# maplant/mgf

Measured on AMD Instinct MI355X. Metric: contact_constraint_iters_per_sec, higher is better.
Workload: dtype f32

## Files before the change

mgf_amd/csrc/common.h:

```cpp
#pragma once
#include <hip/hip_runtime.h>
#include <stdint.h>
#include <stdio.h>
#include <string.h>

#include <string>
#include <vector>

#include "../../include/mgf_hip.h"

namespace mgf {

void set_error(const char* fmt, ...);

#define MGF_HIP_TRY(expr)                                                                  \
  do {                                                                                     \
    hipError_t _e = (expr);                                                                \
    if (_e != hipSuccess) {                                                                \
      mgf::set_error("%s failed: %s (%s:%d)", #expr, hipGetErrorString(_e), __FILE__, __LINE__); \
      return (_e == hipErrorOutOfMemory) ? MGF_ERR_OOM : MGF_ERR_HIP;                      \
    }                                                                                      \
  } while (0)

#define MGF_TRY(expr)                 \
// ... 54 lines not shown
  kWFrontier0 = 0, kWFrontier1 = 1, kWFrontier2 = 2,
  kWStackOverflow = 3,
  kWRowOverflow = 4,
  kWSolverAbort = 5,
  kWGridWide = 6,
  kWFlow5Fail = 7,
  kWTerrainWide = 8,
  kWFlow5MaxBlock = 9,
  kWRevRowOverflow = 10,
  kWNarrowMismatch = 11,
  kWStandbyBar = 12,
  kWSkipGuard = 14,
  kWF6MaxSlots = 16, kWF6MaxForeign = 17, kWF6Fail = 18, kWF6Edges = 19, kWF6EdgesBlock = 20,
  kWGhostCons = 21,
  kWBrickSlow = 22,
  kWLinksTicket = 23,
  kWBigPartsOverflow = 24,
  kWLast = kWBigPartsOverflow
};
constexpr int err_at(FlagWord k) { return (int)k - (int)kWStackOverflow; }

mgf_status prim_exclusive_scan_u32(mgf_ctx* ctx, const uint32_t* in, uint32_t* out, size_t n_plus_1);
mgf_status prim_sort_pairs_u32(mgf_ctx* ctx, const uint32_t* keys_in, uint32_t* keys_out, const uint32_t* vals_in, uint32_t* vals_out, size_t n,
                               unsigned end_bit);

}
```

mgf_amd/csrc/host_tick.inc:

```
enum TerrainPlan { kTerrainNone, kTerrainRows, kTerrainGrid };
static TerrainPlan terrain_plan(const mgf_world* w, bool two_pass) {
  if (two_pass || !w->terrain || w->terrain->m.tree.empty() || !w->n_owned) return kTerrainNone;
  return (w->terrain->grid.ready && !w->terrain_grid_off && !w->opt.terrain_tree && w->obstacles.empty()) ? kTerrainGrid : kTerrainRows;
}
static mgf_status world_integrate(mgf_world* w, float dt, bool complete, bool integrate, bool with_bounds, bool with_terrain_rows = false) {
  mgf_ctx* ctx = w->ctx;
  w->invalidate_tick_caches();
  if (w->n_owned == 0) return MGF_OK;
  SceneBounds* sb = with_bounds ? w->sb.p : nullptr;
  const uint32_t* guard = with_bounds ? w->word(kWSkipGuard) : nullptr;
  int* sb_part = (with_terrain_rows && integrate && with_bounds && !w->opt.no_fused_scene_bounds) ? w->sb_part.p : nullptr;
  w->bounds_cover = sb_part ? w->n_owned : 0u;
  MGF_TRY(w->bpk.ensure(4 * (size_t)std::max(w->n, w->n_owned), ctx->stream));
  w->pack_cover = integrate ? w->n_owned : 0u;
  CellSort cs;
  memset(&cs, 0, sizeof(cs));
  if (sb_part && w->plan.zero_launched && w->plan.n == w->n_owned && w->sbg_valid && w->opt.cells_in_integrate) {
    cs.grid = w->sb_grid.p; cs.shift = kMortonBits - 2 * (int)w->plan.levels; cs.min_frac = (float)w->opt.grid_min_frac_pct * 0.01f;
    cs.cell_of = w->cell_of.p; cs.rank = w->cell_rank.p; cs.cell_cnt = w->cell_cnt.p;
    w->cells_cover = w->n_owned; w->cells_levels = w->plan.levels;
  }
  WideSpec wd;
  memset(&wd, 0, sizeof(wd));
  w->wide_tick_on = false;
// ... 201 lines not shown
  if (w->cap_p == 0) { w->cap_p = std::max(4 * n, 1024u); w->cap_t = std::max(2 * n, 1024u); w->cap_c = std::max(4 * n, 1024u); }
  const uint32_t cap_p = w->cap_p, cap_c = w->cap_c;
  if (cap_p >= (1u << 27)) return fail(MGF_ERR_CAPACITY, "too many broadphase partners (k_count_contacts keeps a list position in 27 bits)");
  uint32_t levels = 4;
  const uint64_t cell_fill = (w->has_capsule && !w->has_compound && !w->opt.cell_fill_set) ? std::min<uint64_t>((uint64_t)w->opt.cell_fill, 8u) : (uint64_t)w->opt.cell_fill;
  while ((double)(cell_fill << (2 * levels)) * (double)w->grid_occupancy < 8.0 * (double)n && levels < (uint32_t)kMortonBits / 2) ++levels;
  const uint32_t cells = 1u << (2 * levels), nblocks = cells / kBlock;
  MGF_TRY(w->cell_of.ensure(n, s)); MGF_TRY(w->cell_rank.ensure(n, s)); MGF_TRY(w->sidx.ensure(n, s)); MGF_TRY(w->brank.ensure(n, s));
  w->list_generic = false;
  w->flow5_ok = true; w->flow5_prepped = false; w->flow6_prepped = false; w->f6_fail_known = false; w->canon_ready = false;
  w->scan_tiles = (uint32_t)(((size_t)std::max(cells, n) + 1 + kScanTile - 1) / kScanTile) + 1;
  MGF_TRY(w->scan_ws.ensure(3 * (2 * (size_t)w->scan_tiles + 2), s));
  MGF_TRY(w->cs_sums.ensure(3 * kCsSumStride, s)); MGF_TRY(w->tcn.ensure(n + 1, s)); MGF_TRY(w->front_cnt.ensure(2 * kTnRegions * kTnCntStride, s));
  MGF_TRY(w->lnodes.ensure(qlevel_offset(levels), s)); MGF_TRY(w->leaves.ensure(n, s));
  MGF_TRY(w->cell_lo.ensure((size_t)cells + 1, s)); MGF_TRY(w->cell_cnt.ensure((size_t)cells + 1, s));
  MGF_TRY(w->sub_lo.ensure(nblocks, s)); MGF_TRY(w->sub_hi.ensure(nblocks, s));
  MGF_TRY(w->sub2_lo.ensure(nblocks / 4 + 1, s)); MGF_TRY(w->sub2_hi.ensure(nblocks / 4 + 1, s));
  const bool rows_done = !early && w->terrain_rows_done;
  MGF_TRY(w->t_cnt.ensure(n + 1, s, rows_done, w->n_owned)); MGF_TRY(w->p_cnt.ensure(n + 1, s));
  MGF_TRY(w->t_off.ensure(n + 1, s)); MGF_TRY(w->p_off.ensure(n + 1, s));
  MGF_TRY(w->cons_nat.ensure(cap_c, s));
  MGF_TRY(links_ensure(w, cap_c));
  MGF_TRY(w->degb.ensure(n + 1, s)); MGF_TRY(w->rev.ensure((size_t)n * w->rev_cap, s));
  const bool bounds_done = !early && w->bounds_cover == n && n > 0;
  w->plan.levels = levels; w->plan.cells = cells; w->plan.n = n; w->plan.cap_c = cap_c; w->plan.solver_follows = solver_follows;
  {
    ZeroList z;
    memset(&z, 0, sizeof(z));
    z.p[0] = w->cell_cnt.p; z.words[0] = cells + 1;
    z.p[1] = w->t_cnt.p; z.words[1] = n + 1;
    if (rows_done) { z.p[1] = w->t_cnt.p + w->n_owned; z.words[1] = n - w->n_owned + 1; }
    z.p[2] = w->degb.p; z.words[2] = n + 1;
    z.p[3] = w->word(kWRevRowOverflow); z.words[3] = 1;
    z.p[4] = w->word(kWRowOverflow); z.words[4] = rows_done ? 0 : 1;
    z.p[5] = w->word(kWGridWide); z.words[5] = 1;
    z.p[6] = w->word(kWTerrainWide); z.words[6] = 1;
    z.p[7] = w->pair_stat.p; z.words[7] = kPairStatWords;
    z.p[16] = w->word(kWBrickSlow); z.words[16] = 1;
    z.p[17] = w->scan_ws.p; z.words[17] = 3 * (2 * w->scan_tiles + 2);
    z.p[18] = w->cs_sums.p; z.words[18] = ((early || !rows_done) ? 3 : 2) * kCsSumStride;
    z.p[20] = w->front_cnt.p; z.words[20] = 2 * kTnRegions * kTnCntStride;
    z.p[21] = w->word(kWBigPartsOverflow); z.words[21] = 1;
    z.p[19] = w->tcn.p; z.words[19] = n + 1;
    w->flow5_zeroed = false; w->flow6_zeroed = false;
    if (solver_follows && w->opt.solver_mode == 6) {
      bool ok = false;
      MGF_TRY(flow6_plan(w, cap_c, w->f6_prep_iters ? w->f6_prep_iters : 10u, &ok));
      if (ok) { flow6_zero_entries(w, cap_c, z, 8); w->flow6_zeroed = true; }
    }
    if (solver_follows && w->opt.solver_mode == 5) {
      bool ok = false;
      MGF_TRY(flow5_plan(w, cap_c, &ok));
      if (ok) { flow5_zero_entries(w, cap_c, z, 8); w->flow5_zeroed = true; }
// ... 213 lines not shown
}
static mgf_status stage_pair_search(mgf_world* w, const CollidePlan& P) {
  const Lbvh T = tick_tree(w, P);
  if (P.two_pass) {
    k_candidates<false><<<8 * xcd_blocks_per(P.n), kBlock, 0, P.s>>>(P.B, P.n, w->n_owned, T, P.M, 1e-3f, w->t_cnt.p, w->p_cnt.p, nullptr, nullptr, nullptr, nullptr, nullptr, nullptr, nullptr);
    LAUNCH_CHECK();
    if (P.n_obs && w->n_owned) {
      k_obstacle_candidates<false><<<nblk(w->n_owned), kBlock, 0, P.s>>>(P.B, w->n_owned, w->d_obs.p, P.n_obs, w->t_cnt.p, nullptr, nullptr, nullptr, nullptr);
      LAUNCH_CHECK();
    }
    return MGF_OK;
  }
  if (P.brick && !w->pair_brick_attr) {
    MGF_HIP_TRY(hipFuncSetAttribute(reinterpret_cast<const void*>(k_pair_brick<true>), hipFuncAttributeMaxDynamicSharedMemorySize, (int)brick_lds_bytes(true, kBrickCap)));
    MGF_HIP_TRY(hipFuncSetAttribute(reinterpret_cast<const void*>(k_pair_brick<false>), hipFuncAttributeMaxDynamicSharedMemorySize, (int)brick_lds_bytes(false, kBrickCap)));
    w->pair_brick_attr = true;
  }
  const uint32_t per_block = kCoopBlock / kCoopLanes;
  const uint32_t grid = 8 * (((P.n + per_block - 1) / per_block + 7) / 8);
  const uint32_t bricks = 8 * ((((1u << (2 * P.levels)) >> 6) + 7) / 8);
  uint32_t* const overflow = w->word(kWRowOverflow);
  uint32_t* const too_wide = w->word(kWGridWide);
  if (P.demo) {}
  else if (P.front_rows && w->has_compound) { MGF_TRY(w->cnt.ensure(P.n + 1, P.s)); k_pair_grid_n<true><<<grid, kCoopBlock, 0, P.s>>>(P.B, P.n, w->n_owned, T, w->sb.p, 1e-3f, w->rows.p, w->p_cnt.p, overflow, too_wide, w->pair_stat.p, P.min_frac, w->cnt.p); }
  else if (P.front_rows) k_pair_grid_n<false><<<grid, kCoopBlock, 0, P.s>>>(P.B, P.n, w->n_owned, T, w->sb.p, 1e-3f, w->rows.p, w->p_cnt.p, overflow, too_wide, w->pair_stat.p, P.min_frac, nullptr);
  else if (P.brick && P.fused) k_pair_brick<true><<<bricks, kCoopBlock, brick_lds_bytes(true, kBrickCap), P.s>>>(P.n, w->n_owned, T, w->rows.p, w->p_cnt.p, overflow, too_wide, w->pair_stat.p, w->word(kWBrickSlow), kBrickCap);
  else if (P.brick) k_pair_brick<false><<<bricks, kCoopBlock, brick_lds_bytes(false, kBrickCap), P.s>>>(P.n, w->n_owned, T, w->rows.p, w->p_cnt.p, overflow, too_wide, w->pair_stat.p, w->word(kWBrickSlow), kBrickCap);
  else if (P.use_grid && P.fused) k_pair_grid<true><<<grid, kCoopBlock, 0, P.s>>>(P.B, P.n, w->n_owned, T, w->sb.p, 1e-3f, w->rows.p, w->p_cnt.p, overflow, too_wide, w->pair_stat.p, P.min_frac);
  else if (P.use_grid) k_pair_grid<false><<<grid, kCoopBlock, 0, P.s>>>(P.B, P.n, w->n_owned, T, w->sb.p, 1e-3f, w->rows.p, w->p_cnt.p, overflow, too_wide, nullptr, P.min_frac);
  else k_pair_rows<<<grid, kCoopBlock, 0, P.s>>>(P.B, P.n, w->n_owned, T, 1e-3f, w->rows.p, w->p_cnt.p, overflow);
  LAUNCH_CHECK();
  if (P.wide_now) {
    PairWide W;
    W.list = w->wide_list.p; W.count = &w->sb.p->pad; W.T = T; W.sb = w->sb.p; W.box = P.grid_box_of; W.pad_abs = 1e-3f; W.min_frac = P.min_frac; W.n = P.n; W.n_owned = w->n_owned;
    W.contacts = (P.fused || P.front_rows) ? 1u : 0u; W.rows_p = w->rows.p; W.p_cnt = w->p_cnt.p; W.overflow = overflow; W.too_wide = too_wide;
    W.pair_stat = (P.fused || P.front_rows) ? w->pair_stat.p : nullptr; W.guard = w->word(kWSkipGuard);
    k_pair_wide<<<kWideCap, kBlock, 0, P.s>>>(P.B, W);
    LAUNCH_CHECK();
  }
  return MGF_OK;
}
static mgf_status contacts_from_rows(mgf_world* w, const CollidePlan& P, float dt) {
// ... 235 lines not shown
  {
    const SceneBounds* sbh = reinterpret_cast<SceneBounds*>(pin + mgf_world::kRbSb);
    float e[3], emax = 0.0f;
    for (int k = 0; k < 3; ++k) { e[k] = ord_f(sbh->hi[k]) - ord_f(sbh->lo[k]); emax = std::max(emax, e[k]); w->h_scene_ext[k] = e[k]; w->h_scene_rmax[k] = ord_f(sbh->rmax[k]); }
    const float mf = (float)w->opt.grid_min_frac_pct * 0.01f;
    float occ = 1.0f;
    const uint32_t P = 2u * std::max(w->plan.levels, 4u), nbh[3] = {(P + 2u) / 3u, (P + 1u) / 3u, P / 3u};
    if (emax > 0.0f && mf > 0.0f) for (int k = 0; k < 3; ++k) if (e[k] < mf * emax) {
      const float wide = std::max(e[k], std::min(mf * emax, 1.36f * w->h_scene_rmax[k] * (float)(1u << nbh[k])));
      occ *= std::max(e[k], 1e-3f * emax) / wide;
    }
    w->grid_occupancy = (occ > 0.0f && occ <= 1.0f) ? std::max(occ, 0.3f) : 1.0f;
  }
  w->wide_last = w->wide_tick_on ? reinterpret_cast<SceneBounds*>(pin + mgf_world::kRbSb)->pad : 0u;
  w->pair_brick_slow = w->ts->brick ? w->ts->word(kWBrickSlow) : 0;
  if (w->ts->brick) {
    if (w->pair_brick_slow * 32 > (uint64_t)w->n + 1024) { w->pair_brick_off = w->pair_brick_backoff; w->pair_brick_backoff = std::min(2u * w->pair_brick_backoff, 1u << 20); }
    else w->pair_brick_backoff = 256;
  }
  w->f6_fail_known = w->flow6_prepped; w->f6_fail_host = w->ts->word(kWF6Fail);
  w->f6_edges_block = w->flow6_prepped ? w->ts->word(kWF6EdgesBlock) : 0u;
  w->rb_fresh = true;
  if (w->ts->word(kWStackOverflow)) return fail(MGF_ERR_CAPACITY, "BVH traversal stack overflow");
  if (w->ts->word(kWBigPartsOverflow)) return fail(MGF_ERR_CAPACITY, "two bodies of many components meet in more than 64 part pairs or a manifold of more than 16 contacts (k_narrow_pairs_big)");
  if (w->ts->word(kWNarrowMismatch)) return fail(MGF_ERR_HIP, "internal error: the broadphase's sphere test and the constraint setup disagree about a contact");
  auto grown = [](uint32_t need) { return (uint32_t)std::min<uint64_t>((uint64_t)need + need / 2 + 1024, 0x7FFFFFF0ull); };
  if (h.fail & kFailSkipped) { *retry = true; return MGF_OK; }
  if (h.fail & kFailRevRow) { w->rev_cap *= 2; *retry = true; }
  if (h.fail & kFailFlow6) {
    const uint32_t slots = w->ts->word(kWF6MaxSlots), foreign = w->ts->word(kWF6MaxForeign);
// ... 102 lines not shown
```

mgf_amd/csrc/host_world.inc:

```
struct WorldOptions {
  int64_t resort_every = -1;
  int64_t grid_min_frac_pct = 50;
  int64_t cell_fill = 16;
  bool cell_fill_set = false;
  int64_t cells_in_integrate = 1;
  int64_t no_fused_scene_bounds = 0;
  int64_t no_fused_terrain_rows = 0;
  int64_t two_pass = 0;
  int64_t terrain_tree = 0;
  int64_t broadphase_tree = 0;
  int64_t pair_brick = 1;
  int64_t no_fused_narrowphase = 0;
  int64_t fused_contacts = 1;
  int64_t front_rows = 1;
  int64_t front_rows_check = 0;
  int64_t side_stream = 1;
  int64_t wide_list = 1;
  int64_t constraint_order = 0;
  int64_t solver_mode = 6;
  int64_t flow_spin_limit = 0;
  int64_t flow_max_blocks = 0;
  int64_t flow_trace = 0;
  int64_t flow5_block = 0;
  int64_t flow5_test_cap = 0;
  int64_t flow6_fcap = 0;
  int64_t flow6_spec_wl = -1;
  int64_t flow6_spec = 0;
  int64_t flow6_poll_waves = 0;
  int64_t flow6_const_lds = 1;
  int64_t flow6_foreign_lds = 1;
  int64_t flow6_quad = 1;
  int64_t flow6_quad_max = -1;
  int64_t flow6_slot_margin = 0;
  int64_t flow6_rec_lds = 1;
  int64_t flow6_nimp_lds = 1;
  int64_t flow6_test_cap = 0;
  int64_t pipeline = 1;
  int64_t readback_kernel = 1;
// ... 51 lines not shown
  bool wide_engaged = false, wide_tick_on = false;
  float wide_ref[3] = {0, 0, 0}, wide_limit[3] = {0, 0, 0};
  float shape_rmax[3] = {0, 0, 0};
  uint32_t wide_hold = 0, wide_last = 0;
  uint64_t n_wide_ticks = 0, n_wide_overflows = 0;
  uint64_t n_path_ticks[7] = {0, 0, 0, 0, 0, 0, 0};
  DBuf<float4> wide_list;
  DBuf<float4> q_bc, q_br;
  DBuf<uint32_t> q_cnt, q_start, q_items, q_large, q_misc, q_off, q_vals;
  DBuf<ParticleIn> q_parts; DBuf<int32_t> q_ign, q_hits; DBuf<float> q_boxes;
  DBuf<MovingIn> q_casts;
  uint32_t q_last_large = 0, q_last_cells = 0;
  float q_last_build_ms = 0.0f, q_last_run_ms = 0.0f;
  bool front_rows_off = false;
  uint64_t pair_brick_slow = 0;
  uint32_t pair_brick_off = 0;
  uint32_t pair_brick_backoff = 256;
  bool pair_brick_attr = false;
  DBuf<float4> sub_lo, sub_hi, sub2_lo, sub2_hi;
  DBuf<uint32_t> cell_lo, cell_cnt;
  DBuf<uint32_t> t_cnt, p_cnt, t_off, p_off, t_cand, t_owner, p_cand, p_owner, rows, rows_t;
  DBuf<uint32_t> flow_arr, flow_arr5;
  DBuf<uint64_t> flow_trace;
  DBuf<uint32_t> brank, f5_shared, f5_gcnt, f5_lslot, f5_wg_cnt;
  DBuf<F5Row> f5_table;
  bool flow5_zeroed = false;
  bool f6_fail_known = false;
  uint32_t f6_fail_host = 0;
  bool f6_standby = false;
  uint32_t f6_edges_block = 0;
  bool links_ready = false;
  bool flow5_ok = false, flow5_prepped = false;
  uint32_t f5_nb = 0, f5_nblocks = 0;
  DBuf<uint4> f6_binfo;
  DBuf<uint32_t> f6_bref, f6_fcnt, f6_fbody, f6_nslots, f6_in_key, f6_in_cnt, f6_out_key, f6_out_val, f6_chan_prefix;
// ... 197 lines not shown
  ctx_release(ctx);
}
extern "C" int64_t mgf_world_len(const mgf_world* w) { return w ? (int64_t)w->n_owned : 0; }

struct OptionEntry { const char* key; int64_t WorldOptions::*field; int64_t lo, hi; const char* range; bool plan, prep; };
static const OptionEntry kOptionTable[] = {
    {"time_solver_kernels", &WorldOptions::time_solver_kernels, 1, 0, nullptr, false, false},
    {"two_pass_candidates", &WorldOptions::two_pass, 1, 0, nullptr, true, false},
    {"broadphase_tree", &WorldOptions::broadphase_tree, 1, 0, nullptr, true, false},
    {"terrain_tree", &WorldOptions::terrain_tree, 1, 0, nullptr, true, false},
    {"no_fused_scene_bounds", &WorldOptions::no_fused_scene_bounds, 1, 0, nullptr, true, false},
    {"no_fused_terrain_rows", &WorldOptions::no_fused_terrain_rows, 1, 0, nullptr, true, false},
    {"grid_min_frac_pct", &WorldOptions::grid_min_frac_pct, 0, 100, "grid_min_frac_pct: 0..100", true, false},
    {"no_fused_narrowphase", &WorldOptions::no_fused_narrowphase, 1, 0, nullptr, false, false},
    {"pair_brick", &WorldOptions::pair_brick, 1, 0, nullptr, false, false},
    {"fused_contacts", &WorldOptions::fused_contacts, 1, 0, nullptr, false, false},
    {"front_rows", &WorldOptions::front_rows, 1, 0, nullptr, false, false},
    {"front_rows_check", &WorldOptions::front_rows_check, 1, 0, nullptr, false, false},
    {"side_stream", &WorldOptions::side_stream, 1, 0, nullptr, false, false},
    {"cells_in_integrate", &WorldOptions::cells_in_integrate, 1, 0, nullptr, false, false},
    {"solver_mode", &WorldOptions::solver_mode, 1, 0, nullptr, false, true},
    {"flow_trace", &WorldOptions::flow_trace, 1, 0, nullptr, false, false},
    {"flow_spin_limit", &WorldOptions::flow_spin_limit, 0, 4 << 20, "flow_spin_limit: 0 .. 4194304", false, false},
    {"flow5_test_cap", &WorldOptions::flow5_test_cap, 1, 0, nullptr, false, false},
    {"flow6_fcap", &WorldOptions::flow6_fcap, 0, 1536, "flow6_fcap out of range", false, false},
    {"flow6_const_lds", &WorldOptions::flow6_const_lds, 1, 0, nullptr, false, false},
    {"flow6_foreign_lds", &WorldOptions::flow6_foreign_lds, 1, 0, nullptr, false, false},
    {"flow6_nimp_lds", &WorldOptions::flow6_nimp_lds, 1, 0, nullptr, false, false},
    {"flow6_rec_lds", &WorldOptions::flow6_rec_lds, 1, 0, nullptr, false, false},
    {"flow6_slot_margin", &WorldOptions::flow6_slot_margin, 0, 1024, "flow6_slot_margin: 0..1024", false, false},
// ... 61 lines not shown
      w->has_compound = true;
    }
    return MGF_OK;
  }
  if (!strcmp(key, "list_capacity")) {
    if (value < 1 || value > 0x7FFFFFF0ll) return fail(MGF_ERR_INVALID, "list_capacity out of range");
    w->cap_t = w->cap_p = w->cap_c = (uint32_t)value;
    return MGF_OK;
  }
  return fail(MGF_ERR_INVALID, "unknown option");
}

extern "C" mgf_status mgf_world_counter(const mgf_world* w, const char* name, int64_t* out) {
  if (!w || !name || !out) return fail(MGF_ERR_INVALID, "NULL argument");
  if (!strcmp(name, "pair_brick_slow_queries")) { *out = (int64_t)w->pair_brick_slow; return MGF_OK; }
  if (!strcmp(name, "pair_brick_off_ticks")) { *out = (int64_t)w->pair_brick_off; return MGF_OK; }
  if (!strncmp(name, "scene_rmax_milli_", 17) && name[17] >= 'x' && name[17] <= 'z' && !name[18]) { *out = (int64_t)std::ceil((double)w->h_scene_rmax[name[17] - 'x'] * 1000.0); return MGF_OK; }
  if (!strncmp(name, "scene_ext_milli_", 16) && name[16] >= 'x' && name[16] <= 'z' && !name[17]) { *out = (int64_t)std::ceil((double)w->h_scene_ext[name[16] - 'x'] * 1000.0); return MGF_OK; }
  if (!strcmp(name, "grid_levels")) { *out = (int64_t)w->plan.levels; return MGF_OK; }
  if (!strcmp(name, "max_fat_half_extent_x_milli")) { *out = (int64_t)std::ceil((double)w->last_rmax_x * 1000.0); return MGF_OK; }
  if (!strncmp(name, "cross_probe_", 12)) {
    *out = 0;
    mgf_world* mw = const_cast<mgf_world*>(w);
    const size_t n = w->n;
    if (!w->constraints_ready || w->C == 0 || n == 0) return MGF_OK;
    MGF_TRY(ctx_bind(mw->ctx));
    std::vector<float4> x(n);
    MGF_TRY(d2h(mw->ctx, x.data(), mw->x.p, n));
    float lo[3] = {3e38f, 3e38f, 3e38f}, hi[3] = {-3e38f, -3e38f, -3e38f};
    for (const float4& v : x) { const float c[3] = {v.x, v.y, v.z}; for (int k = 0; k < 3; ++k) { lo[k] = std::min(lo[k], c[k]); hi[k] = std::max(hi[k], c[k]); } }
// ... 594 lines not shown
```

mgf_amd/csrc/k_broadphase.h:

```cpp
#pragma once
#include "k_bodies.h"

namespace mgf {

__device__ __forceinline__ uint32_t expand10(uint32_t v) {
  v = (v * 0x00010001u) & 0xFF0000FFu;
  v = (v * 0x00000101u) & 0x0F00F00Fu;
  v = (v * 0x00000011u) & 0xC30C30C3u;
  v = (v * 0x00000005u) & 0x49249249u;
  return v;
}
__device__ __forceinline__ uint32_t morton_quant(float v, float lo, float hi) {
  float ext = hi - lo;
  float t = ext > 0.0f ? (v - lo) / ext : 0.0f;
  int qv = (int)(t * 1023.0f);
  return (uint32_t)(qv < 0 ? 0 : (qv > 1023 ? 1023 : qv));
}
__device__ __forceinline__ uint32_t face_cell(uint32_t cx, uint32_t cy, uint32_t cz, uint3 bits) {
  return (((cx << bits.y) | cy) << bits.z) | cz;
}
constexpr int kMortonBits = 30;
constexpr float kBodyGridMinFrac = 0.5f;
__device__ __forceinline__ void grid_box(const SceneBounds* sb, float min_frac, uint32_t P, float* lo, float* hi) {
  float ext = 0.0f;
// ... 1022 lines not shown
    if (!SPHERES && np > (uint32_t)kRowCap) atomicOr(overflow, 1u);
  }
  if (SPHERES) {
    __shared__ uint32_t s_sum;
    if (threadIdx.x == 0) s_sum = 0;
    __syncthreads();
    uint32_t v = (live && sub == 0) ? n_accepted : 0u;
#pragma unroll
    for (int o = 32; o >= 1; o >>= 1) v += __shfl_xor(v, o);
    if (lane == 0 && v) atomicAdd(&s_sum, v);
    __syncthreads();
    if (threadIdx.x == 0 && s_sum) atomicAdd(&pair_stat[blockIdx.x & (kPairStatWords - 1u)], s_sum);
  }
}

template <bool SPHERES>
__global__ __launch_bounds__(kCoopBlock) __attribute__((amdgpu_waves_per_eu(6, 8))) void k_pair_brick(uint32_t n, uint32_t n_owned, Lbvh T,
                                                           uint32_t* rows_p, uint32_t* p_cnt, uint32_t* overflow, uint32_t* too_wide,
                                                           uint32_t* pair_stat, uint32_t* slow_queries, uint32_t cap) {
  extern __shared__ float4 s_dyn[];
  __shared__ uint16_t s_start[516];
  __shared__ uint32_t s_wsum[kCoopBlock / 64];
  __shared__ uint16_t s_acc[SPHERES ? kBrickQueries : 1][SPHERES ? kRowCap : 1];
  __shared__ uint32_t s_cnt[kBrickQueries][3];
  __shared__ uint32_t s_qo[kBrickQueries];
  __shared__ uint32_t s_sum, s_slow, s_q[2];
  const uint32_t P = 2u * T.levels;
  const uint32_t nbricks = (1u << P) >> 6;
  const uint32_t brick = xcd_logical_block_coop();
  if (brick >= nbricks) return;
  const uint32_t nb[3] = {(P + 2u) / 3u, (P + 1u) / 3u, P / 3u};
  const int shift = kMortonBits - (int)P;
  BrickSrcLds L;
  const uint32_t capp = brick_phys_cap(cap);
// ... 17 lines not shown
    }
  }
  if (t == 0) { s_sum = 0; s_slow = 0; }
  uint32_t inc = cnt;
#pragma unroll
  for (int o = 1; o < 64; o <<= 1) { uint32_t u = __shfl_up(inc, o); if (lane >= o) inc += u; }
  if (lane == 63) s_wsum[t >> 6] = inc;
  if (t == ((2u << 6) | (2u << 3) | 2u)) s_q[0] = g0;
  if (t == ((5u << 6) | (5u << 3) | 5u)) s_q[1] = g0 + cnt;
  __syncthreads();
  const uint32_t q0 = s_q[0], q1 = s_q[1];
  if (q0 == q1) return;
  uint32_t base = 0, total = 0;
#pragma unroll
  for (int w = 0; w < kCoopBlock / 64; ++w) { const uint32_t u = s_wsum[w]; if (w < (int)(t >> 6)) base += u; total += u; }
  const uint32_t start = base + inc - cnt;
  const bool staged = total <= cap;
  s_start[t] = (uint16_t)min(start, 0xFFFFu);
  if (t == 0) { s_start[512] = (uint16_t)min(total, 0xFFFFu); s_start[513] = s_start[512]; }
  uint32_t kq = q0 + t / (uint32_t)kBrickLanes;
  float4 qc, qr, qa, qv;
  qc = qr = qa = qv = make_float4(0, 0, 0, 0);
  uint32_t qi = 0;
  uint2 qreg = make_uint2(0, 0);
  if (kq < q1) { qc = T.ltb[2 * kq]; qr = T.ltb[2 * kq + 1]; if (SPHERES) { qa = T.lcol[2 * kq]; qv = T.lcol[2 * kq + 1]; } qi = T.sidx[kq]; qreg = make_uint2(f2u(qc.w), f2u(qr.w)); }
  if ((t & (uint32_t)(kBrickLanes - 1)) == 0u) s_qo[t / (uint32_t)kBrickLanes] = kq < q1 ? f2u(T.leaves[kq].r.w) : 0u;
  if (staged) {
    float4* rc = s_dyn; float4* rr = s_dyn + capp; float4* cc = s_dyn + 2 * capp; float4* cd = s_dyn + 3 * capp;
    for (uint32_t r = 0; r < cnt; ++r) {
      LeafRec lr = T.leaves[g0 + r];
      const uint32_t pp = brick_phys(start + r);
      rc[pp] = lr.c; rr[pp] = lr.r;
      if (SPHERES) { cc[pp] = T.lcol[2 * (g0 + r)]; cd[pp] = T.lcol[2 * (g0 + r) + 1]; }
    }
  }
  __syncthreads();
  const uint32_t sub = t & (uint32_t)(kBrickLanes - 1), qg = t / (uint32_t)kBrickLanes;
  uint32_t acc_total = 0, slow = 0;
  for (;;) {
    const bool live = kq < q1;
    const uint32_t i = qi, oi = s_qo[qg];
    uint32_t np = 0;
    if (sub == 0) { s_cnt[qg][0] = 0; s_cnt[qg][1] = 0; s_cnt[qg][2] = 0; }
    __builtin_amdgcn_fence(__ATOMIC_ACQ_REL, "wavefront");
    if (live && oi != 0 && T.n >= 2) {
      Box q; q.c = xyz(qc); q.r = xyz(qr);
      Comp A; A.p = xyz(qa); A.r = qa.w; A.d = mk3(0, 0, 0); A.kind = KIND_SPHERE;
      const V3 vA = xyz(qv);
      const uint32_t ca[3] = {qreg.x & 1023u, (qreg.x >> 10) & 1023u, qreg.x >> 20}, d[3] = {qreg.y & 1023u, (qreg.y >> 10) & 1023u, qreg.y >> 20};
      uint32_t* row = rows_p + (size_t)i * kRowCap;
      if (d[0] * d[1] * d[2] > kGridMaxCells) {
        if (sub == 0) *too_wide = 1u;
      } else if (staged && (int)ca[0] >= L.hb[0] && (int)ca[1] >= L.hb[1] && (int)ca[2] >= L.hb[2] && (int)(ca[0] + d[0]) <= L.hb[0] + 8 &&
                 (int)(ca[1] + d[1]) <= L.hb[1] + 8 && (int)(ca[2] + d[2]) <= L.hb[2] + 8) {
        brick_query<SPHERES>(L, q, A, vA, oi, n_owned, ca, d, sub, (uint32_t)kBrickLanes, row, s_acc[SPHERES ? qg : 0], s_cnt[qg]);
      } else if (sub == 0) {
        BrickSrcGlobal S; S.T = T; S.nb[0] = nb[0]; S.nb[1] = nb[1]; S.nb[2] = nb[2]; S.shift = shift;
        brick_query<SPHERES>(S, q, A, vA, oi, n_owned, ca, d, 0u, 1u, row, row, s_cnt[qg]);
        ++slow;
      }
      __builtin_amdgcn_fence(__ATOMIC_ACQ_REL, "wavefront");
      const uint32_t accepted = *(volatile uint32_t*)&s_cnt[qg][0];
      np = SPHERES ? *(volatile uint32_t*)&s_cnt[qg][2] : accepted;
      if (sub == 0) {
        acc_total += accepted;
        if (accepted > (uint32_t)kRowCap) atomicOr(overflow, 1u);
      }
    }
    if (live && sub == 0) p_cnt[i] = np;
    kq += kBrickQueries;
    if (kq - qg >= q1) break;
    qi = 0;
    if (kq < q1) { qc = T.ltb[2 * kq]; qr = T.ltb[2 * kq + 1]; if (SPHERES) { qa = T.lcol[2 * kq]; qv = T.lcol[2 * kq + 1]; } qi = T.sidx[kq]; qreg = make_uint2(f2u(qc.w), f2u(qr.w)); }
    if (sub == 0) s_qo[qg] = kq < q1 ? f2u(T.leaves[kq].r.w) : 0u;
  }
  {
    uint32_t v = acc_total, u = slow;
#pragma unroll
    for (int o = 32; o >= 1; o >>= 1) { v += __shfl_xor(v, o); u += __shfl_xor(u, o); }
    if (lane == 0 && v) atomicAdd(&s_sum, v);
    if (lane == 0 && u) atomicAdd(&s_slow, u);
    __syncthreads();
    if (SPHERES && t == 0 && s_sum) atomicAdd(&pair_stat[blockIdx.x & (kPairStatWords - 1u)], s_sum);
    if (t == 0 && s_slow) atomicAdd(slow_queries, s_slow);
  }
}
constexpr size_t brick_lds_bytes(bool spheres, uint32_t cap) { return (size_t)brick_phys_cap(cap) * 16u * (spheres ? 4u : 2u); }

struct FaceGrid {
  Lbvh T;
  uint3 bits;
  const SceneBounds* sb;
  const uint32_t* rank_of_face;
  const uint32_t* leaf_of_face;
  const uint32_t* parent;
};
__global__ __launch_bounds__(kCoopBlock) void k_terrain_grid(Bodies B, uint32_t n_owned, const uint32_t* order, TerrainDev M, FaceGrid G,
                                                             float pad_abs, uint32_t cap_row, uint32_t* rows_t, uint32_t* t_cnt,
                                                             uint32_t* overflow, uint32_t* too_wide) {
  const int lane = threadIdx.x & 63;
  const int sub = lane & 7;
// ... 132 lines not shown
```

Before: 8.422 billion.

## Split overfull bricks into sub-brick LDS passes instead of per-lane global fallback

Bricks whose staged leaf count exceeds LDS capacity no longer fall back to slow single-lane global-memory queries. They are appended to an overflow list and handled by a second kernel. That kernel splits each brick into Morton sub-ranges small enough to stage in LDS and serves their queries cooperatively. The cost is an extra kernel launch every tick, more counter words, and added complexity in the sub-range partitioning.

```diff
diff --git a/mgf_amd/csrc/common.h b/mgf_amd/csrc/common.h
--- a/mgf_amd/csrc/common.h
+++ b/mgf_amd/csrc/common.h
@@ -92,8 +92,11 @@
   kWF6MaxSlots = 16, kWF6MaxForeign = 17, kWF6Fail = 18, kWF6Edges = 19, kWF6EdgesBlock = 20,
   kWGhostCons = 21,
   kWBrickSlow = 22,
-  kWLinksTicket = 23,
-  kWBigPartsOverflow = 24,
+  kWBrickSplit = 23,
+  kWBrickLane = 24,
+  kWBrickOver = 25,
+  kWLinksTicket = 26,
+  kWBigPartsOverflow = 27,
   kWLast = kWBigPartsOverflow
 };
 constexpr int err_at(FlagWord k) { return (int)k - (int)kWStackOverflow; }
diff --git a/mgf_amd/csrc/host_tick.inc b/mgf_amd/csrc/host_tick.inc
--- a/mgf_amd/csrc/host_tick.inc
+++ b/mgf_amd/csrc/host_tick.inc
@@ -239,6 +239,7 @@
   MGF_TRY(w->cs_sums.ensure(3 * kCsSumStride, s)); MGF_TRY(w->tcn.ensure(n + 1, s)); MGF_TRY(w->front_cnt.ensure(2 * kTnRegions * kTnCntStride, s));
   MGF_TRY(w->lnodes.ensure(qlevel_offset(levels), s)); MGF_TRY(w->leaves.ensure(n, s));
   MGF_TRY(w->cell_lo.ensure((size_t)cells + 1, s)); MGF_TRY(w->cell_cnt.ensure((size_t)cells + 1, s));
+  MGF_TRY(w->brick_over.ensure((size_t)cells / 64 + 8, s));
   MGF_TRY(w->sub_lo.ensure(nblocks, s)); MGF_TRY(w->sub_hi.ensure(nblocks, s));
   MGF_TRY(w->sub2_lo.ensure(nblocks / 4 + 1, s)); MGF_TRY(w->sub2_hi.ensure(nblocks / 4 + 1, s));
   const bool rows_done = !early && w->terrain_rows_done;
@@ -261,7 +262,7 @@
     z.p[5] = w->word(kWGridWide); z.words[5] = 1;
     z.p[6] = w->word(kWTerrainWide); z.words[6] = 1;
     z.p[7] = w->pair_stat.p; z.words[7] = kPairStatWords;
-    z.p[16] = w->word(kWBrickSlow); z.words[16] = 1;
+    z.p[16] = w->word(kWBrickSlow); z.words[16] = 4;
     z.p[17] = w->scan_ws.p; z.words[17] = 3 * (2 * w->scan_tiles + 2);
     z.p[18] = w->cs_sums.p; z.words[18] = ((early || !rows_done) ? 3 : 2) * kCsSumStride;
     z.p[20] = w->front_cnt.p; z.words[20] = 2 * kTnRegions * kTnCntStride;
@@ -505,18 +506,27 @@
   if (P.brick && !w->pair_brick_attr) {
     MGF_HIP_TRY(hipFuncSetAttribute(reinterpret_cast<const void*>(k_pair_brick<true>), hipFuncAttributeMaxDynamicSharedMemorySize, (int)brick_lds_bytes(true, kBrickCap)));
     MGF_HIP_TRY(hipFuncSetAttribute(reinterpret_cast<const void*>(k_pair_brick<false>), hipFuncAttributeMaxDynamicSharedMemorySize, (int)brick_lds_bytes(false, kBrickCap)));
+    MGF_HIP_TRY(hipFuncSetAttribute(reinterpret_cast<const void*>(k_pair_brick_split<true>), hipFuncAttributeMaxDynamicSharedMemorySize, (int)brick_lds_bytes(true, kBrickCap)));
+    MGF_HIP_TRY(hipFuncSetAttribute(reinterpret_cast<const void*>(k_pair_brick_split<false>), hipFuncAttributeMaxDynamicSharedMemorySize, (int)brick_lds_bytes(false, kBrickCap)));
     w->pair_brick_attr = true;
   }
   const uint32_t per_block = kCoopBlock / kCoopLanes;
   const uint32_t grid = 8 * (((P.n + per_block - 1) / per_block + 7) / 8);
   const uint32_t bricks = 8 * ((((1u << (2 * P.levels)) >> 6) + 7) / 8);
+  static_assert(kWBrickSplit == kWBrickSlow + 1 && kWBrickLane == kWBrickSlow + 2 && kWBrickOver == kWBrickSlow + 3, "k_pair_brick and k_pair_brick_split count into four consecutive words");
+  const uint32_t brick_cap = w->opt.pair_brick_test_cap > 0 ? (uint32_t)std::min<int64_t>(w->opt.pair_brick_test_cap, (int64_t)kBrickCap) : kBrickCap;
   uint32_t* const overflow = w->word(kWRowOverflow);
   uint32_t* const too_wide = w->word(kWGridWide);
   if (P.demo) {}
   else if (P.front_rows && w->has_compound) { MGF_TRY(w->cnt.ensure(P.n + 1, P.s)); k_pair_grid_n<true><<<grid, kCoopBlock, 0, P.s>>>(P.B, P.n, w->n_owned, T, w->sb.p, 1e-3f, w->rows.p, w->p_cnt.p, overflow, too_wide, w->pair_stat.p, P.min_frac, w->cnt.p); }
   else if (P.front_rows) k_pair_grid_n<false><<<grid, kCoopBlock, 0, P.s>>>(P.B, P.n, w->n_owned, T, w->sb.p, 1e-3f, w->rows.p, w->p_cnt.p, overflow, too_wide, w->pair_stat.p, P.min_frac, nullptr);
-  else if (P.brick && P.fused) k_pair_brick<true><<<bricks, kCoopBlock, brick_lds_bytes(true, kBrickCap), P.s>>>(P.n, w->n_owned, T, w->rows.p, w->p_cnt.p, overflow, too_wide, w->pair_stat.p, w->word(kWBrickSlow), kBrickCap);
-  else if (P.brick) k_pair_brick<false><<<bricks, kCoopBlock, brick_lds_bytes(false, kBrickCap), P.s>>>(P.n, w->n_owned, T, w->rows.p, w->p_cnt.p, overflow, too_wide, w->pair_stat.p, w->word(kWBrickSlow), kBrickCap);
+  else if (P.brick && P.fused) {
+    k_pair_brick<true><<<bricks, kCoopBlock, brick_lds_bytes(true, kBrickCap), P.s>>>(P.n, w->n_owned, T, w->rows.p, w->p_cnt.p, overflow, too_wide, w->pair_stat.p, w->word(kWBrickSlow), brick_cap, w->brick_over.p);
+    k_pair_brick_split<true><<<std::min(bricks, kBrickSplitBlocks), kCoopBlock, brick_lds_bytes(true, kBrickCap), P.s>>>(w->n_owned, T, w->rows.p, w->p_cnt.p, overflow, too_wide, w->pair_stat.p, w->word(kWBrickSlow), brick_cap, w->brick_over.p);
+  } else if (P.brick) {
+    k_pair_brick<false><<<bricks, kCoopBlock, brick_lds_bytes(false, kBrickCap), P.s>>>(P.n, w->n_owned, T, w->rows.p, w->p_cnt.p, overflow, too_wide, w->pair_stat.p, w->word(kWBrickSlow), brick_cap, w->brick_over.p);
+    k_pair_brick_split<false><<<std::min(bricks, kBrickSplitBlocks), kCoopBlock, brick_lds_bytes(false, kBrickCap), P.s>>>(w->n_owned, T, w->rows.p, w->p_cnt.p, overflow, too_wide, w->pair_stat.p, w->word(kWBrickSlow), brick_cap, w->brick_over.p);
+  }
   else if (P.use_grid && P.fused) k_pair_grid<true><<<grid, kCoopBlock, 0, P.s>>>(P.B, P.n, w->n_owned, T, w->sb.p, 1e-3f, w->rows.p, w->p_cnt.p, overflow, too_wide, w->pair_stat.p, P.min_frac);
   else if (P.use_grid) k_pair_grid<false><<<grid, kCoopBlock, 0, P.s>>>(P.B, P.n, w->n_owned, T, w->sb.p, 1e-3f, w->rows.p, w->p_cnt.p, overflow, too_wide, nullptr, P.min_frac);
   else k_pair_rows<<<grid, kCoopBlock, 0, P.s>>>(P.B, P.n, w->n_owned, T, 1e-3f, w->rows.p, w->p_cnt.p, overflow);
@@ -782,6 +792,8 @@
   }
   w->wide_last = w->wide_tick_on ? reinterpret_cast<SceneBounds*>(pin + mgf_world::kRbSb)->pad : 0u;
   w->pair_brick_slow = w->ts->brick ? w->ts->word(kWBrickSlow) : 0;
+  w->pair_brick_split = w->ts->brick ? w->ts->word(kWBrickSplit) : 0;
+  w->pair_brick_lane = w->ts->brick ? w->ts->word(kWBrickLane) : 0;
   if (w->ts->brick) {
     if (w->pair_brick_slow * 32 > (uint64_t)w->n + 1024) { w->pair_brick_off = w->pair_brick_backoff; w->pair_brick_backoff = std::min(2u * w->pair_brick_backoff, 1u << 20); }
     else w->pair_brick_backoff = 256;
diff --git a/mgf_amd/csrc/host_world.inc b/mgf_amd/csrc/host_world.inc
--- a/mgf_amd/csrc/host_world.inc
+++ b/mgf_amd/csrc/host_world.inc
@@ -22,6 +22,7 @@
   int64_t flow_max_blocks = 0;
   int64_t flow_trace = 0;
   int64_t flow5_block = 0;
+  int64_t pair_brick_test_cap = 0;
   int64_t flow5_test_cap = 0;
   int64_t flow6_fcap = 0;
   int64_t flow6_spec_wl = -1;
@@ -103,11 +104,14 @@
   float q_last_build_ms = 0.0f, q_last_run_ms = 0.0f;
   bool front_rows_off = false;
   uint64_t pair_brick_slow = 0;
+  uint64_t pair_brick_split = 0;
+  uint64_t pair_brick_lane = 0;
   uint32_t pair_brick_off = 0;
   uint32_t pair_brick_backoff = 256;
   bool pair_brick_attr = false;
   DBuf<float4> sub_lo, sub_hi, sub2_lo, sub2_hi;
   DBuf<uint32_t> cell_lo, cell_cnt;
+  DBuf<uint32_t> brick_over;
   DBuf<uint32_t> t_cnt, p_cnt, t_off, p_off, t_cand, t_owner, p_cand, p_owner, rows, rows_t;
   DBuf<uint32_t> flow_arr, flow_arr5;
   DBuf<uint64_t> flow_trace;
@@ -335,6 +339,7 @@
     {"grid_min_frac_pct", &WorldOptions::grid_min_frac_pct, 0, 100, "grid_min_frac_pct: 0..100", true, false},
     {"no_fused_narrowphase", &WorldOptions::no_fused_narrowphase, 1, 0, nullptr, false, false},
     {"pair_brick", &WorldOptions::pair_brick, 1, 0, nullptr, false, false},
+    {"pair_brick_test_cap", &WorldOptions::pair_brick_test_cap, 1, 0, nullptr, false, false},
     {"fused_contacts", &WorldOptions::fused_contacts, 1, 0, nullptr, false, false},
     {"front_rows", &WorldOptions::front_rows, 1, 0, nullptr, false, false},
     {"front_rows_check", &WorldOptions::front_rows_check, 1, 0, nullptr, false, false},
@@ -426,6 +431,8 @@
 extern "C" mgf_status mgf_world_counter(const mgf_world* w, const char* name, int64_t* out) {
   if (!w || !name || !out) return fail(MGF_ERR_INVALID, "NULL argument");
   if (!strcmp(name, "pair_brick_slow_queries")) { *out = (int64_t)w->pair_brick_slow; return MGF_OK; }
+  if (!strcmp(name, "pair_brick_split_queries")) { *out = (int64_t)w->pair_brick_split; return MGF_OK; }
+  if (!strcmp(name, "pair_brick_lane_queries")) { *out = (int64_t)w->pair_brick_lane; return MGF_OK; }
   if (!strcmp(name, "pair_brick_off_ticks")) { *out = (int64_t)w->pair_brick_off; return MGF_OK; }
   if (!strncmp(name, "scene_rmax_milli_", 17) && name[17] >= 'x' && name[17] <= 'z' && !name[18]) { *out = (int64_t)std::ceil((double)w->h_scene_rmax[name[17] - 'x'] * 1000.0); return MGF_OK; }
   if (!strncmp(name, "scene_ext_milli_", 16) && name[16] >= 'x' && name[16] <= 'z' && !name[17]) { *out = (int64_t)std::ceil((double)w->h_scene_ext[name[16] - 'x'] * 1000.0); return MGF_OK; }
diff --git a/mgf_amd/csrc/k_broadphase.h b/mgf_amd/csrc/k_broadphase.h
--- a/mgf_amd/csrc/k_broadphase.h
+++ b/mgf_amd/csrc/k_broadphase.h
@@ -1060,10 +1060,87 @@
   }
 }
 
+__device__ __forceinline__ void brick_box(uint32_t brick, const uint32_t* nb, int shift, int* hb) {
+  const uint32_t code = (brick * 64u) << shift;
+  hb[0] = (int)(compact10(code >> 2) >> (10u - nb[0])) - 2;
+  hb[1] = (int)(compact10(code >> 1) >> (10u - nb[1])) - 2;
+  hb[2] = (int)(compact10(code) >> (10u - nb[2])) - 2;
+}
+__device__ __forceinline__ void brick_own_cell(const Lbvh& T, const int* hb, const uint32_t* nb, int shift, uint32_t t, uint32_t& g0, uint32_t& cnt) {
+  const int c[3] = {hb[0] + (int)(t >> 6), hb[1] + (int)((t >> 3) & 7u), hb[2] + (int)(t & 7u)};
+  g0 = 0; cnt = 0;
+  if (c[0] >= 0 && c[1] >= 0 && c[2] >= 0 && c[0] < (1 << nb[0]) && c[1] < (1 << nb[1]) && c[2] < (1 << nb[2])) {
+    const uint32_t cd = (expand10((uint32_t)c[0] << (10u - nb[0])) << 2) | (expand10((uint32_t)c[1] << (10u - nb[1])) << 1) |
+                        expand10((uint32_t)c[2] << (10u - nb[2]));
+    g0 = T.cell_lo[cd >> shift];
+    cnt = T.cell_lo[(size_t)(cd >> shift) + 1] - g0;
+  }
+}
+struct BrickQ { float4 qc, qr, qa, qv; uint32_t qi; uint2 qreg; };
+template <bool SPHERES>
+__device__ __forceinline__ void brick_fetch(const Lbvh& T, uint32_t kq, uint32_t pb, uint32_t sub, BrickQ& Q, uint32_t* qo_g) {
+  Q.qi = 0;
+  if (kq < pb) { Q.qc = T.ltb[2 * kq]; Q.qr = T.ltb[2 * kq + 1]; if (SPHERES) { Q.qa = T.lcol[2 * kq]; Q.qv = T.lcol[2 * kq + 1]; } Q.qi = T.sidx[kq]; Q.qreg = make_uint2(f2u(Q.qc.w), f2u(Q.qr.w)); }
+  if (sub == 0u) *qo_g = kq < pb ? f2u(T.leaves[kq].r.w) : 0u;
+}
+template <bool SPHERES>
+__device__ __forceinline__ void brick_stage(const Lbvh& T, float4* s_dyn, uint32_t capp, uint32_t g0, uint32_t cnt, uint32_t start) {
+  float4* rc = s_dyn; float4* rr = s_dyn + capp; float4* cc = s_dyn + 2 * capp; float4* cd = s_dyn + 3 * capp;
+  for (uint32_t r = 0; r < cnt; ++r) {
+    LeafRec lr = T.leaves[g0 + r];
+    const uint32_t pp = brick_phys(start + r);
+    rc[pp] = lr.c; rr[pp] = lr.r;
+    if (SPHERES) { cc[pp] = T.lcol[2 * (g0 + r)]; cd[pp] = T.lcol[2 * (g0 + r) + 1]; }
+  }
+}
+constexpr uint32_t kWholeBox = 0x888000u;
+template <bool SPHERES>
+__device__ __forceinline__ void brick_serve(const BrickSrcLds& L, const Lbvh& T, const uint32_t* nb, int shift, uint32_t n_owned, uint32_t* rows_p, uint32_t* p_cnt,
+                                            uint32_t* overflow, uint32_t* too_wide, uint32_t kq, uint32_t pb, uint32_t pbox, BrickQ& Q, uint32_t sub, uint32_t qg,
+                                            uint16_t* acc_g, uint32_t* cnt_g, uint32_t* qo_g, uint32_t& acc_total, uint32_t& lane_q, uint32_t& lds_q) {
+  for (;;) {
+    const bool live = kq < pb;
+    const uint32_t i = Q.qi, oi = *qo_g;
+    uint32_t np = 0;
+    if (sub == 0) { cnt_g[0] = 0; cnt_g[1] = 0; cnt_g[2] = 0; }
+    __builtin_amdgcn_fence(__ATOMIC_ACQ_REL, "wavefront");
+    if (live && oi != 0 && T.n >= 2) {
+      Box q; q.c = xyz(Q.qc); q.r = xyz(Q.qr);
+      Comp A; A.p = xyz(Q.qa); A.r = Q.qa.w; A.d = mk3(0, 0, 0); A.kind = KIND_SPHERE;
+      const V3 vA = xyz(Q.qv);
+      const uint32_t ca[3] = {Q.qreg.x & 1023u, (Q.qreg.x >> 10) & 1023u, Q.qreg.x >> 20}, d[3] = {Q.qreg.y & 1023u, (Q.qreg.y >> 10) & 1023u, Q.qreg.y >> 20};
+      uint32_t* row = rows_p + (size_t)i * kRowCap;
+      if (d[0] * d[1] * d[2] > kGridMaxCells) {
+        if (sub == 0) *too_wide = 1u;
+      } else if ((int)ca[0] >= L.hb[0] + (int)(pbox & 15u) && (int)ca[1] >= L.hb[1] + (int)((pbox >> 4) & 15u) && (int)ca[2] >= L.hb[2] + (int)((pbox >> 8) & 15u) &&
+                 (int)(ca[0] + d[0]) <= L.hb[0] + (int)((pbox >> 12) & 15u) && (int)(ca[1] + d[1]) <= L.hb[1] + (int)((pbox >> 16) & 15u) &&
+                 (int)(ca[2] + d[2]) <= L.hb[2] + (int)(pbox >> 20)) {
+        brick_query<SPHERES>(L, q, A, vA, oi, n_owned, ca, d, sub, (uint32_t)kBrickLanes, row, acc_g, cnt_g);
+        if (sub == 0) ++lds_q;
+      } else if (sub == 0) {
+        BrickSrcGlobal S; S.T = T; S.nb[0] = nb[0]; S.nb[1] = nb[1]; S.nb[2] = nb[2]; S.shift = shift;
+        brick_query<SPHERES>(S, q, A, vA, oi, n_owned, ca, d, 0u, 1u, row, row, cnt_g);
+        ++lane_q;
+      }
+      __builtin_amdgcn_fence(__ATOMIC_ACQ_REL, "wavefront");
+      const uint32_t accepted = *(volatile uint32_t*)&cnt_g[0];
+      np = SPHERES ? *(volatile uint32_t*)&cnt_g[2] : accepted;
+      if (sub == 0) {
+        acc_total += accepted;
+        if (accepted > (uint32_t)kRowCap) atomicOr(overflow, 1u);
+      }
+    }
+    if (live && sub == 0) p_cnt[i] = np;
+    kq += kBrickQueries;
+    if (kq - qg >= pb) break;
+    brick_fetch<SPHERES>(T, kq, pb, sub, Q, qo_g);
+  }
+}
+
 template <bool SPHERES>
 __global__ __launch_bounds__(kCoopBlock) __attribute__((amdgpu_waves_per_eu(6, 8))) void k_pair_brick(uint32_t n, uint32_t n_owned, Lbvh T,
                                                            uint32_t* rows_p, uint32_t* p_cnt, uint32_t* overflow, uint32_t* too_wide,
-                                                           uint32_t* pair_stat, uint32_t* slow_queries, uint32_t cap) {
+                                                           uint32_t* pair_stat, uint32_t* slow_queries, uint32_t cap, uint32_t* over_list) {
   extern __shared__ float4 s_dyn[];
   __shared__ uint16_t s_start[516];
   __shared__ uint32_t s_wsum[kCoopBlock / 64];
@@ -1111,8 +1188,11 @@
   uint32_t base = 0, total = 0;
 #pragma unroll
   for (int w = 0; w < kCoopBlock / 64; ++w) { const uint32_t u = s_wsum[w]; if (w < (int)(t >> 6)) base += u; total += u; }
+  if (total > cap) {
+    if (t == 0) over_list[atomicAdd(slow_queries + 3, 1u)] = brick;
+    return;
+  }
   const uint32_t start = base + inc - cnt;
-  const bool staged = total <= cap;
   s_start[t] = (uint16_t)min(start, 0xFFFFu);
   if (t == 0) { s_start[512] = (uint16_t)min(total, 0xFFFFu); s_start[513] = s_start[512]; }
   uint32_t kq = q0 + t / (uint32_t)kBrickLanes;
@@ -1122,7 +1202,7 @@
   uint2 qreg = make_uint2(0, 0);
   if (kq < q1) { qc = T.ltb[2 * kq]; qr = T.ltb[2 * kq + 1]; if (SPHERES) { qa = T.lcol[2 * kq]; qv = T.lcol[2 * kq + 1]; } qi = T.sidx[kq]; qreg = make_uint2(f2u(qc.w), f2u(qr.w)); }
   if ((t & (uint32_t)(kBrickLanes - 1)) == 0u) s_qo[t / (uint32_t)kBrickLanes] = kq < q1 ? f2u(T.leaves[kq].r.w) : 0u;
-  if (staged) {
+  {
     float4* rc = s_dyn; float4* rr = s_dyn + capp; float4* cc = s_dyn + 2 * capp; float4* cd = s_dyn + 3 * capp;
     for (uint32_t r = 0; r < cnt; ++r) {
       LeafRec lr = T.leaves[g0 + r];
@@ -1148,7 +1228,7 @@
       uint32_t* row = rows_p + (size_t)i * kRowCap;
       if (d[0] * d[1] * d[2] > kGridMaxCells) {
         if (sub == 0) *too_wide = 1u;
-      } else if (staged && (int)ca[0] >= L.hb[0] && (int)ca[1] >= L.hb[1] && (int)ca[2] >= L.hb[2] && (int)(ca[0] + d[0]) <= L.hb[0] + 8 &&
+      } else if ((int)ca[0] >= L.hb[0] && (int)ca[1] >= L.hb[1] && (int)ca[2] >= L.hb[2] && (int)(ca[0] + d[0]) <= L.hb[0] + 8 &&
                  (int)(ca[1] + d[1]) <= L.hb[1] + 8 && (int)(ca[2] + d[2]) <= L.hb[2] + 8) {
         brick_query<SPHERES>(L, q, A, vA, oi, n_owned, ca, d, sub, (uint32_t)kBrickLanes, row, s_acc[SPHERES ? qg : 0], s_cnt[qg]);
       } else if (sub == 0) {
@@ -1179,9 +1259,98 @@
     if (lane == 0 && u) atomicAdd(&s_slow, u);
     __syncthreads();
     if (SPHERES && t == 0 && s_sum) atomicAdd(&pair_stat[blockIdx.x & (kPairStatWords - 1u)], s_sum);
-    if (t == 0 && s_slow) atomicAdd(slow_queries, s_slow);
-  }
-}
+    if (t == 0 && s_slow) { atomicAdd(slow_queries, s_slow); atomicAdd(slow_queries + 2, s_slow); }
+  }
+}
+template <bool SPHERES>
+__global__ __launch_bounds__(kCoopBlock) void k_pair_brick_split(uint32_t n_owned, Lbvh T, uint32_t* rows_p, uint32_t* p_cnt, uint32_t* overflow, uint32_t* too_wide,
+                                                                 uint32_t* pair_stat, uint32_t* slow_queries, uint32_t cap, const uint32_t* over_list) {
+  extern __shared__ float4 s_dyn[];
+  __shared__ uint16_t s_start[516];
+  __shared__ uint32_t s_wsum[kCoopBlock / 64];
+  __shared__ uint16_t s_acc[SPHERES ? kBrickQueries : 1][SPHERES ? kRowCap : 1];
+  __shared__ uint32_t s_cnt[kBrickQueries][3];
+  __shared__ uint32_t s_qo[kBrickQueries];
+  __shared__ uint32_t s_sum, s_lane, s_split;
+  const uint32_t n_over = slow_queries[3];
+  if (blockIdx.x >= n_over) return;
+  const uint32_t P = 2u * T.levels;
+  const uint32_t nb[3] = {(P + 2u) / 3u, (P + 1u) / 3u, P / 3u};
+  const int shift = kMortonBits - (int)P;
+  BrickSrcLds L;
+  const uint32_t capp = brick_phys_cap(cap);
+  L.rc = s_dyn; L.rr = s_dyn + capp; L.cc = s_dyn + 2 * capp; L.cd = s_dyn + 3 * capp; L.start = s_start;
+  const uint32_t t = threadIdx.x;
+  const int lane = t & 63;
+  const uint32_t sub = t & (uint32_t)(kBrickLanes - 1), qg = t / (uint32_t)kBrickLanes;
+  const uint32_t tc[3] = {t >> 6, (t >> 3) & 7u, t & 7u};
+  if (t == 0) { s_sum = 0; s_lane = 0; s_split = 0; }
+  uint32_t acc_total = 0, lane_q = 0, lds_q = 0;
+  for (uint32_t k = blockIdx.x; k < n_over; k += gridDim.x) {
+    const uint32_t brick = over_list[k];
+    brick_box(brick, nb, shift, L.hb);
+    uint32_t g0, cnt;
+    brick_own_cell(T, L.hb, nb, shift, t, g0, cnt);
+    const uint32_t* clo = T.cell_lo + (size_t)brick * 64u;
+    for (uint32_t e = 0; e < 8u;) {
+      if (clo[8u * e] == clo[8u * e + 8u]) { ++e; continue; }
+      uint32_t sz = (e & 3u) == 0u ? 4u : (e & 1u) == 0u ? 2u : 1u;
+      uint32_t pbox = 0, pcnt = 0, pstart = 0;
+      for (;;) {
+        const uint32_t ma = (8u * e) << shift, mb = (8u * (e + sz) - 1u) << shift;
+        const uint32_t lo[3] = {compact10(ma >> 2) >> (10u - nb[0]), compact10(ma >> 1) >> (10u - nb[1]), compact10(ma) >> (10u - nb[2])};
+        const uint32_t hi[3] = {(compact10(mb >> 2) >> (10u - nb[0])) + 5u, (compact10(mb >> 1) >> (10u - nb[1])) + 5u, (compact10(mb) >> (10u - nb[2])) + 5u};
+        const bool in = tc[0] >= lo[0] && tc[0] < hi[0] && tc[1] >= lo[1] && tc[1] < hi[1] && tc[2] >= lo[2] && tc[2] < hi[2];
+        pcnt = in ? cnt : 0u;
+        uint32_t pinc = pcnt;
+#pragma unroll
+        for (int o = 1; o < 64; o <<= 1) { uint32_t u = __shfl_up(pinc, o); if (lane >= o) pinc += u; }
+        __syncthreads();
+        if (lane == 63) s_wsum[t >> 6] = pinc;
+        __syncthreads();
+        uint32_t pbase = 0, ptotal = 0;
+#pragma unroll
+        for (int w = 0; w < kCoopBlock / 64; ++w) { const uint32_t u = s_wsum[w]; if (w < (int)(t >> 6)) pbase += u; ptotal += u; }
+        ptotal = (uint32_t)__builtin_amdgcn_readfirstlane((int)ptotal);
+        if (ptotal <= cap) {
+          pbox = lo[0] | (lo[1] << 4) | (lo[2] << 8) | (hi[0] << 12) | (hi[1] << 16) | (hi[2] << 20);
+          pstart = pbase + pinc - pcnt;
+          s_start[t] = (uint16_t)pstart;
+          if (t == 0) { s_start[512] = (uint16_t)ptotal; s_start[513] = (uint16_t)ptotal; }
+          break;
+        }
+        if (sz == 1u) { pcnt = 0; break; }
+        sz >>= 1;
+      }
+      const uint32_t kq = clo[8u * e] + qg, pb = clo[8u * (e + sz)];
+      e += sz;
+      BrickQ Q;
+      Q.qc = Q.qr = Q.qa = Q.qv = make_float4(0, 0, 0, 0); Q.qreg = make_uint2(0, 0);
+      brick_fetch<SPHERES>(T, kq, pb, sub, Q, &s_qo[qg]);
+      brick_stage<SPHERES>(T, s_dyn, capp, g0, pcnt, pstart);
+      __syncthreads();
+      brick_serve<SPHERES>(L, T, nb, shift, n_owned, rows_p, p_cnt, overflow, too_wide, kq, pb, pbox, Q, sub, qg, s_acc[SPHERES ? qg : 0], s_cnt[qg], &s_qo[qg],
+                           acc_total, lane_q, lds_q);
+    }
+  }
+  {
+    uint32_t v = acc_total, u = lane_q, x = lds_q;
+#pragma unroll
+    for (int o = 32; o >= 1; o >>= 1) { v += __shfl_xor(v, o); u += __shfl_xor(u, o); x += __shfl_xor(x, o); }
+    __syncthreads();
+    if (lane == 0 && v) atomicAdd(&s_sum, v);
+    if (lane == 0 && u) atomicAdd(&s_lane, u);
+    if (lane == 0 && x) atomicAdd(&s_split, x);
+    __syncthreads();
+    if (SPHERES && t == 0 && s_sum) atomicAdd(&pair_stat[blockIdx.x & (kPairStatWords - 1u)], s_sum);
+    if (t == 0 && (s_lane | s_split)) {
+      atomicAdd(slow_queries, s_lane + s_split);
+      if (s_split) atomicAdd(slow_queries + 1, s_split);
+      if (s_lane) atomicAdd(slow_queries + 2, s_lane);
+    }
+  }
+}
+constexpr uint32_t kBrickSplitBlocks = 512;
 constexpr size_t brick_lds_bytes(bool spheres, uint32_t cap) { return (size_t)brick_phys_cap(cap) * 16u * (spheres ? 4u : 2u); }
 
 struct FaceGrid {
```

Result: no change. 8.375 billion (-0.6%).
